# ltdoanh2004/MotionDiffusion-MoE

Hardware: AMD Instinct MI355X
Metric: denoising-steps/sec (B=32, T=196, 263-d, 8 experts) (higher is better)
Workload: dtype bf16; 1 GPU; configs[1]: model_size=small, num_experts=8, B=32/GPU, T=196, 1000-step DDPM with CFG 7.5 (cond+uncond batched as 64 rows), N_text=28, hipGraph=on, streams=1; global_batch=32, parallelism=batch-shard x1, weights replicated

## Files before the change

### include/mdm_hip.h

```cpp
#ifndef MDM_HIP_H
#define MDM_HIP_H
#include <stdint.h>

#ifdef __cplusplus
extern "C" {
#endif

enum { MDM_OK = 0, MDM_ERR_ARG = 1, MDM_ERR_LAUNCH = 2, MDM_ERR_UNSUPPORTED = 3 };
enum { MDM_OP_F32_ROW = 0, MDM_OP_F32_KSTRIDE = 1, MDM_OP_BF16_ROW = 2, MDM_OP_FP8_ROW = 3 ,
       MDM_OP_X2_ROW = 4 };
enum { MDM_ACT_NONE = 0, MDM_ACT_GELU = 1, MDM_ACT_SILU = 2, MDM_ACT_FEAT = 3,
       MDM_ACT_HEADNORM = 4,
       MDM_ACT_HEADSOFTMAX = 5 };
enum { MDM_H16_BF16 = 1, MDM_H16_F16 = 2 };
enum { MDM_PREC_BF16 = 1, MDM_PREC_F16 = 2, MDM_PREC_X3 = 3, MDM_PREC_MIXED = 4, MDM_PREC_FP8 = 5 };

typedef struct MdmOperand {
  const void* p;
  const void* p_lo;
  int64_t ld;
  int64_t gstride;
  const int32_t* gather;
  int64_t bs1, bs2;
  int32_t rpg;
// ... 378 lines not shown
  float* w1;
  float* b1;
  float* w2;
  float* b2;
  float* st_emb_w;
  float* st_emb_b;
  float* st_norm_w;
  float* st_norm_b;
  float* st_out_w;
  float* st_out_b;
} MdmMoeTensors;

int64_t mdm_moe_train_workspace_bytes(int32_t B, int32_t S, int32_t D, int32_t F, int32_t E, int32_t Te);
int mdm_moe_ffn_train_forward(const MdmMoeTensors* params, int32_t D, int32_t F, int32_t E, int32_t Te, int32_t De,
                              const float* eph_w, const float* eph_b, const float* x, const float* emb, int32_t B, int32_t S,
                              float dropout_p, uint64_t seed, float* out, float* lb_loss, int32_t* route_out, void* ws,
                              int64_t ws_bytes, void* stream);
int mdm_moe_ffn_train_backward(const MdmMoeTensors* params, int32_t D, int32_t F, int32_t E, int32_t Te, int32_t De,
                               const float* eph_w, const float* x, const float* emb, int32_t B, int32_t S, float dropout_p,
                               uint64_t seed, const float* dout, float* dx, float* demb, const MdmMoeTensors* grads, void* ws,
                               int64_t ws_bytes, void* stream);
int mdm_sumsq(const float* x, int64_t n, float* out, void* stream);
int mdm_adam_step(float* p, const float* g, float* m, float* v, int64_t n, float lr, float beta1, float beta2, float eps,
                  int32_t step, const float* sumsq, float max_norm, void* stream);

int mdm_xattn_gate(const float* gate, const float* adaptive_gate, int32_t D, float* out, void* stream);
int mdm_fill_i64(int64_t* dst, int64_t n, const int32_t* src_dev, void* stream);
int mdm_add_i32(int32_t* dst, int32_t delta, void* stream);

enum MdmVariant {
  MDM_VAR_DEFAULT = 0,
  MDM_VAR_GEMM_256 = 6,
  MDM_VAR_SD_UNFOLDED = 22,
  MDM_VAR_GENERIC_DH256 = 23,
  MDM_VAR_SD_FOLD_ANY = 24,
  MDM_VAR_ROUTER_CONST_E = 26,
  MDM_VAR_ROUTER_RUNTIME_E = 27,
  MDM_VAR_MLP_LDS = 34,
  MDM_VAR_TAIL_SPLIT = 35,
  MDM_VAR_X3_REG = 36,
  MDM_VAR_QKV_SPLIT = 50,
  MDM_VAR_XQ_SPLIT = 51,
  MDM_VAR_X3_ATTN_CHAIN = 52,
  MDM_VAR_X3_XATTN_CHAIN = 56,
  MDM_VAR_X3_STYLE_SPLIT = 60,
  MDM_VAR_X3_TAILS_SPLIT = 61,
  MDM_VAR_X3_F32_ROWS = 62,
  MDM_VAR_STREAM_NEVER = 63,
  MDM_VAR_STREAM_ALWAYS = 68,
  MDM_VAR_STREAM3_NEVER = 69,
  MDM_VAR_STREAM3_ALWAYS = 70
};
enum MdmRouteVariant { MDM_VAR_ROUTE_LAUNCH = 171 };
int mdm_set_gemm_variant(int variant);

int mdm_probe_enable(int32_t enable);
int mdm_route_dump(int32_t* buf, int64_t capacity);
int mdm_route_workspace(const MdmModel* m, int32_t B, int32_t T, int32_t N, int64_t* off);
int mdm_sd_fold_passes(int32_t D, int32_t H, int32_t N);
int mdm_probe_read(float* us, int32_t* rows, int32_t cap);


int64_t mdm_gru_bidir_workspace_bytes(int32_t B, int32_t H);
int mdm_gru_bidir(const float* gx, const float* w_hh, const float* b_hh, const float* h0, const int32_t* lens_dev,
                  const int32_t* lens_host, int32_t B, int32_t T, int32_t H, float* out, float* ws, int64_t ws_bytes, void* stream);
int mdm_eval_pad_rows(const float* src, int64_t ld_src, int32_t B, int32_t T, int32_t C, int32_t Cp, int32_t pad, int32_t leaky,
                      float* dst, void* stream);
int mdm_eval_ln_leaky(const float* x, int32_t M, int32_t N, const float* w, const float* b, float eps, float* y, void* stream);
int mdm_eval_matching(const float* text, const float* motion, int32_t B, int32_t D, float* dist, int32_t* rank, float* diag,
                      void* stream);
int mdm_eval_center(const float* x, int32_t N, int32_t D, float* mean, float* xc, void* stream);

const char* mdm_version(void);

#ifdef __cplusplus
}
#endif
#endif
```

### motiondiffusion-moe_amd/csrc/api.hip

```cpp
#include "gemm.h"
#include "kernels.h"

namespace mdm {
namespace {

__global__ void pack_bf16_kernel(const float* __restrict__ src, int64_t ld_src, int64_t rows, int64_t K,
                                 uint16_t* __restrict__ hi, uint16_t* __restrict__ lo, int64_t ld_dst) {
  const int64_t pairs_per_row = ld_dst >> 1;
  const int64_t total = rows * pairs_per_row;
  for (int64_t i = blockIdx.x * (int64_t)blockDim.x + threadIdx.x; i < total; i += (int64_t)gridDim.x * blockDim.x) {
    const int64_t r = i / pairs_per_row, k = (i - r * pairs_per_row) * 2;
    const float a = k < K ? src[r * ld_src + k] : 0.f;
    const float b = k + 1 < K ? src[r * ld_src + k + 1] : 0.f;
    uint32_t h, l;
    split_bf16(a, b, h, l);
    *(uint32_t*)(hi + r * ld_dst + k) = h;
    if (lo) *(uint32_t*)(lo + r * ld_dst + k) = l;
  }
}

__global__ void pack_f16_kernel(const float* __restrict__ src, int64_t ld_src, int64_t rows, int64_t K,
                                uint16_t* __restrict__ dst, int64_t ld_dst) {
  const int64_t pairs_per_row = ld_dst >> 1;
  const int64_t total = rows * pairs_per_row;
  for (int64_t i = blockIdx.x * (int64_t)blockDim.x + threadIdx.x; i < total; i += (int64_t)gridDim.x * blockDim.x) {
    const int64_t r = i / pairs_per_row, k = (i - r * pairs_per_row) * 2;
    const float a = k < K ? src[r * ld_src + k] : 0.f;
    const float b = k + 1 < K ? src[r * ld_src + k + 1] : 0.f;
    *(uint32_t*)(dst + r * ld_dst + k) = pack_f16(a, b);
  }
}

}
}

namespace mdm {
int g_variant = MDM_VAR_DEFAULT;
}

extern "C" {

int mdm_set_gemm_variant(int v) {
  switch (v) {
    case MDM_VAR_DEFAULT:
    case MDM_VAR_GEMM_256:
    case MDM_VAR_SD_UNFOLDED:
    case MDM_VAR_GENERIC_DH256:
    case MDM_VAR_SD_FOLD_ANY:
    case MDM_VAR_ROUTER_CONST_E:
    case MDM_VAR_ROUTER_RUNTIME_E:
    case MDM_VAR_MLP_LDS:
    case MDM_VAR_TAIL_SPLIT:
    case MDM_VAR_X3_REG:
    case MDM_VAR_QKV_SPLIT:
    case MDM_VAR_XQ_SPLIT:
    case MDM_VAR_X3_ATTN_CHAIN:
    case MDM_VAR_X3_XATTN_CHAIN:
    case MDM_VAR_X3_STYLE_SPLIT:
    case MDM_VAR_X3_TAILS_SPLIT:
    case MDM_VAR_X3_F32_ROWS:
    case MDM_VAR_STREAM_NEVER:
    case MDM_VAR_STREAM_ALWAYS:
    case MDM_VAR_STREAM3_NEVER:
    case MDM_VAR_STREAM3_ALWAYS:
    case MDM_VAR_ROUTE_LAUNCH:
      mdm::g_variant = v;
      return MDM_OK;
    default:
      return MDM_ERR_ARG;
  }
}

const char* mdm_version(void) { return "mdm_hip 0.1 (gfx950)"; }

int mdm_gemm(const MdmGemmDesc* d, void* stream) {
  if (!d) return MDM_ERR_ARG;
  return mdm::gemm(*d, (hipStream_t)stream);
}

int mdm_fused_mlp(const MdmMlpDesc* d, void* stream) {
  if (!d) return MDM_ERR_ARG;
  return mdm::fused_mlp(*d, (hipStream_t)stream);
}

int64_t mdm_mlp_stream_elems(int32_t G, int32_t F, int32_t Din, int32_t Dout) { return mdm::mlp_stream_elems(G, F, Din, Dout); }

int mdm_mlp_stream_pack(const float* w1, const float* w2, int32_t G, int32_t F, int32_t Din, int32_t Dout, int32_t h16,
                        uint16_t* out, void* stream) {
  return mdm::mlp_stream_pack(w1, w2, G, F, Din, Dout, h16, out, (hipStream_t)stream);
}

int64_t mdm_gemm_stream_elems(int32_t N, int32_t K) { return mdm::gemm_stream_elems(N, K); }

int mdm_gemm_stream_pack(const float* w, int32_t N, int32_t K, int32_t h16, uint16_t* out, void* stream) {
  return mdm::gemm_stream_pack(w, N, K, h16, out, (hipStream_t)stream);
}

int64_t mdm_gemm_stream1_elems(int32_t N, int32_t K) { return mdm::gemm_stream1_elems(N, K); }

int mdm_gemm_stream1_pack(const float* w, int64_t ldw, int32_t N, int32_t K, int32_t h16, uint16_t* out, void* stream) {
  return mdm::gemm_stream1_pack(w, ldw, N, K, h16, out, (hipStream_t)stream);
}

int64_t mdm_gemm_stream3x_elems(int32_t G, int32_t N, int32_t K) { return mdm::gemm_stream3x_elems(G, N, K); }

int64_t mdm_gemm_stream3x_group_elems(int32_t N, int32_t K) { return mdm::gemm_stream3x_group_elems(N, K); }

int mdm_gemm_stream3x_pack(const float* w, int64_t ldw, int32_t G, int32_t N, int32_t K, uint16_t* out, void* stream) {
  return mdm::gemm_stream3x_pack(w, ldw, G, N, K, out, (hipStream_t)stream);
}

int64_t mdm_gemm_stream3_elems(int32_t N, int32_t K) { return mdm::gemm_stream3_elems(N, K); }

int mdm_gemm_stream3_pack(const float* w, int32_t N, int32_t K, uint16_t* out, void* stream) {
  return mdm::gemm_stream3_pack(w, N, K, out, (hipStream_t)stream);
}

int mdm_pack_bf16(const float* src, int64_t ld_src, int64_t rows, int64_t K, uint16_t* hi, uint16_t* lo,
// ... 35 lines not shown
```

### motiondiffusion-moe_amd/csrc/gemm.h

```cpp
#pragma once
#include "mdm_common.h"
#include "mdm_hip.h"

namespace mdm {

typedef MdmOperand Operand;
typedef MdmGemmDesc GemmArgs;

enum OperandKind { OP_F32_ROW = MDM_OP_F32_ROW, OP_F32_KSTRIDE = MDM_OP_F32_KSTRIDE, OP_BF16_ROW = MDM_OP_BF16_ROW, OP_X2_ROW = MDM_OP_X2_ROW };
enum Act { ACT_NONE = MDM_ACT_NONE, ACT_GELU = MDM_ACT_GELU, ACT_SILU = MDM_ACT_SILU, ACT_FEAT = MDM_ACT_FEAT, ACT_HEADNORM = MDM_ACT_HEADNORM, ACT_HEADSOFTMAX = MDM_ACT_HEADSOFTMAX };

inline GemmArgs gemm_defaults(int precision) {
  GemmArgs g = {};
  g.batch = 1;
  g.nb2 = 1;
  g.alpha = 1.f;
  g.out_scale = 1.f;
  g.r1_scale = 1.f;
  g.precision = precision;
  g.a_scale_u = 1.f;
  g.c8_scale = 1.f;
  return g;
}
inline Operand op_f32(const float* p, int64_t ld) {
  Operand o = {};
  o.p = p;
  o.ld = ld;
  o.kind = OP_F32_ROW;
  return o;
}
inline Operand op_f32_kstride(const float* p, int64_t ld) {
  Operand o = {};
  o.p = p;
  o.ld = ld;
  o.kind = OP_F32_KSTRIDE;
  return o;
}
inline Operand op_bf16(const uint16_t* hi, const uint16_t* lo, int64_t ld) {
  Operand o = {};
  o.p = hi;
  o.p_lo = lo;
  o.ld = ld;
  o.kind = OP_BF16_ROW;
  return o;
}

int gemm(const GemmArgs& a, hipStream_t stream);
bool gemm_bf16_eligible(const GemmArgs& a);
int gemm_bf16(const GemmArgs& a, hipStream_t stream);
bool gemm_bf16_256_eligible(const GemmArgs& a);
int gemm_bf16_256(const GemmArgs& a, hipStream_t stream);
bool fused_mlp_supported(const MdmMlpDesc& a);
int fused_mlp(const MdmMlpDesc& a, hipStream_t stream);
bool gemm_x3_dma_eligible(const GemmArgs& a);
int gemm_x3_dma(const GemmArgs& a, hipStream_t stream);
bool gemm_fp8_eligible(const GemmArgs& a);
int gemm_fp8(const GemmArgs& a, hipStream_t stream);
int64_t gemm_stream1_elems(int N, int K);
int gemm_stream1_pack(const float* w, int64_t ldw, int N, int K, int h16, uint16_t* out, hipStream_t stream);
bool gemm_stream1_eligible(const GemmArgs& a);
bool gemm_stream1_wanted(const GemmArgs& a);
int gemm_stream1(const GemmArgs& a, hipStream_t stream);
int64_t gemm_stream3x_elems(int G, int N, int K);
int64_t gemm_stream3x_group_elems(int N, int K);
int gemm_stream3x_pack(const float* w, int64_t ldw, int G, int N, int K, uint16_t* out, hipStream_t stream);
bool gemm_stream3x_eligible(const GemmArgs& a);
bool gemm_stream3x_wanted(const GemmArgs& a);
int gemm_stream3x(const GemmArgs& a, hipStream_t stream);
bool fused_mlp_stream_supported(const MdmMlpDesc& a);
int fused_mlp_stream(const MdmMlpDesc& a, hipStream_t stream);
struct PairTail {
  const float *pw, *pb;
  const float *sw, *sb;
  const float* sc;
  int S;
  const uint16_t* ws;
  const float* bias;
  const float* resid;
  float out_scale;
  float* out;
  const float *lw, *lb;
  uint16_t* ln16;
  const float* skip;
  float skip_scale;
  const float *l2w, *l2b;
};
bool fused_pair_style_supported(const MdmMlpDesc& a);
int fused_pair_style(const MdmMlpDesc& a, const PairTail& t, hipStream_t stream);
int64_t mlp_stream_elems(int G, int F, int Din, int Dout);
int mlp_stream_pack(const float* w1, const float* w2, int G, int F, int Din, int Dout, int h16, uint16_t* out, hipStream_t stream);
int64_t gemm_stream_elems(int N, int K);
int gemm_stream_pack(const float* w, int N, int K, int h16, uint16_t* out, hipStream_t stream);
bool style_gemm_supported(int D, int64_t M);
int64_t gemm_stream3_elems(int N, int K);
int gemm_stream3_pack(const float* w, int N, int K, uint16_t* out, hipStream_t stream);
struct StyleTail3 {
  const float *lw = nullptr, *lb = nullptr;
  float* ln_out = nullptr;
  const float* skip = nullptr;
  float skip_scale = 0.f;
  const float *l2w = nullptr, *l2b = nullptr;
  int ln_x2 = 0;
};
struct MoeGateParams;
struct StyleRoute {
  const MoeGateParams* gate = nullptr;
  int E = 0;
  int* cursor = nullptr;
};
bool style_gemm_route_supported(int D, int64_t M, int E, int hn_fmt, int h16);
int64_t style_gemm_route_parts(int64_t M);
int style_gemm3(const float* src, int64_t M, int D, int S, const float* pw, const float* pb, const float* sw, const float* sb,
                const float* sc, const int* pos4, const uint16_t* ws3, const float* bias, const float* resid, float out_scale,
                const float* colscale, float* out, const StyleTail3& t, hipStream_t s);
int style_gemm(const void* src, int src_fmt, int64_t M, int D, int S, const float* pw, const float* pb, const float* sw, const float* sb,
               const float* sc, const int* pos4, const uint16_t* ws, const float* bias, const float* resid, float out_scale,
               const float* colscale, float* out, uint16_t* out16, int h16, hipStream_t s, const StyleRoute* route = nullptr);

}
```

### motiondiffusion-moe_amd/csrc/mlp_stream.hip

```cpp
#include <utility>

#include "gemm.h"
#include "kernels.h"
#include "row.h"

namespace mdm {
namespace {

constexpr int NT = 512, FC = 256;

template <typename T>
__device__ __forceinline__ T ldg(const uint8_t* p) {
  return *(const T*)p;
}

__device__ __forceinline__ void pin() { __builtin_amdgcn_sched_barrier(0); }

__device__ __forceinline__ void lds_barrier() {
  asm volatile("s_waitcnt lgkmcnt(0)" ::: "memory");
  __builtin_amdgcn_s_barrier();
  asm volatile("" ::: "memory");
}

__device__ __forceinline__ bool find_tile(const MdmMlpDesc& g, const int* gtab, int tile_h, int lane, int mt, int& row0, int& row_end,
// ... 243 lines not shown
    for (int i = 0; i < RT; ++i) {
      const int ml = i * 16 + frow;
      f32x4 v = y[i][j];
      v[0] = (v[0] + bb[0]) * st.out_scale, v[1] = (v[1] + bb[1]) * st.out_scale, v[2] = (v[2] + bb[2]) * st.out_scale,
      v[3] = (v[3] + bb[3]) * st.out_scale;
      *(f32x4*)(stg + ml * D + (((n >> 2) ^ (ml & 31)) << 2)) = v;
    }
  }
  lds_barrier();
  {
    R8 xr[RPW], sk[RPW];
#pragma unroll
    for (int q = 0; q < RPW; ++q) {
      int64_t m = (int64_t)row0 + RPW * wn + q;
      m = m < row_end ? m : row_end - 1;
      xr[q].load(st.resid + m * D, D, lane);
      if (st.skip) sk[q].load(st.skip + m * D, D, lane);
    }
    R8 lww, lbb, l2ww, l2bb;
    if (st.lw) lww.load(st.lw, D, lane), lbb.load(st.lb, D, lane);
    if (st.l2w) l2ww.load(st.l2w, D, lane), l2bb.load(st.l2b, D, lane);
#pragma unroll
    for (int q = 0; q < RPW; ++q) {
      const int rl = RPW * wn + q;
      const int64_t m = (int64_t)row0 + rl;
      if (m >= row_end) continue;
      R8 r;
      const R8& x = xr[q];
      const f32x4 v0 = *(const f32x4*)(stg + rl * D + ((lane ^ (rl & 31)) << 2));
      const f32x4 v1 = *(const f32x4*)(stg + rl * D + (((64 + lane) ^ (rl & 31)) << 2));
      r.e[0] = v0[0] + x.e[0], r.e[1] = v0[1] + x.e[1], r.e[2] = v0[2] + x.e[2], r.e[3] = v0[3] + x.e[3];
      r.e[4] = v1[0] + x.e[4], r.e[5] = v1[1] + x.e[5], r.e[6] = v1[2] + x.e[6], r.e[7] = v1[3] + x.e[7];
      if (st.skip) {
#pragma unroll
        for (int j = 0; j < 8; ++j) r.e[j] = sk[q].e[j] + st.skip_scale * r.e[j];
        r.layernorm(lww, lbb, D, lane);
        r.store(st.out + m * D, D, lane);
        if (st.l2w) {
          r.layernorm(l2ww, l2bb, D, lane);
          r.template store_h16<FMT>(st.ln16 + m * D, D, lane);
        }
      } else {
        r.store(st.out + m * D, D, lane);
        if (st.ln16) {
          r.layernorm(lww, lbb, D, lane);
          r.template store_h16<FMT>(st.ln16 + m * D, D, lane);
        }
      }
    }
  }
}

template <typename HT, int RT, int NJ, int DIN, int TAIL>
__global__ __launch_bounds__(NT, 2) void fused_mlp_stream_kernel(const MdmMlpDesc g, const int tile_h, const PairTail st) {
  typedef typename HT::frag_t frag_t;
  static_assert(!TAIL || (NJ == 4 && DIN == 512 && RT <= 4), "the tail is written for D = 512 rows");
  typedef XGeo<RT, DIN, NJ, TAIL != 0> G;
  constexpr int NKO = DIN / 128, NLINE = DIN / 64;
  constexpr int NA = 4, PD = NA - 1;
  constexpr int NR = (RT <= 4 && NJ == 4 && DIN % 256 == 0) ? 16 : 8;
  constexpr int NF = 4 * RT;
  static_assert(NF % NA == 0, "the ring must close over the unrolled body");
  extern __shared__ __attribute__((aligned(1024))) uint8_t smem[];
  uint8_t* const ximg = smem;
  uint8_t* const hid = smem + G::XIMG_B;
  int* const gtab = (int*)(smem + G::SMEM);
  {
    const int ng = g.goff ? g.ngroups : 1;
    if ((int)threadIdx.x <= ng) gtab[threadIdx.x] = g.goff ? g.goff[threadIdx.x] : (threadIdx.x ? g.M : 0);
    lds_barrier();
  }

  for (int mt = xcd_remap(blockIdx.x, gridDim.x);; mt += gridDim.x) {
    int tid = threadIdx.x;
    asm volatile("" : "+v"(tid));
    const int lane = tid & 63;
    const int wn = __builtin_amdgcn_readfirstlane(tid >> 6);
    int row0, row_end, grp;
    if (!find_tile(g, gtab, tile_h, lane, mt, row0, row_end, grp)) break;

    const int nchunk = g.F / FC;
    constexpr int fpc = (DIN / 32) * 2 + 8 * NJ;
    const uint8_t* wp = (const uint8_t*)g.wstream + ((int64_t)grp * g.wstream_gs + (int64_t)wn * nchunk * fpc * 512) * 2 + lane * 16;

    frag_t R[NR];
#pragma unroll
    for (int f = 0; f < NR; ++f) R[f] = ldg<frag_t>(wp + f * 1024);
    wp += NR * 1024;

    if (wn < RT) {
      const uint8_t* xp[2];
#pragma unroll
      for (int hf = 0; hf < 2; ++hf) {
        const int r = 16 * wn + 8 * hf + (lane >> 3);
        int srow = row0 + r;
        srow = srow < row_end ? srow : row_end - 1;
        const int64_t src = g.gather ? (int64_t)g.gather[srow] : (int64_t)srow;
        xp[hf] = (const uint8_t*)(g.X + src * g.ldx) + (lane & 7) * 16;
      }
      constexpr int LB = NLINE < 8 ? NLINE : 8;
#pragma unroll
      for (int c0 = 0; c0 < NLINE; c0 += LB) {
        uint4 v[2][LB];
#pragma unroll
        for (int c = 0; c < LB; ++c)
#pragma unroll
          for (int hf = 0; hf < 2; ++hf) v[hf][c] = ldg<uint4>(xp[hf] + (c0 + c) * 128);
#pragma unroll
        for (int c = 0; c < LB; ++c)
#pragma unroll
          for (int hf = 0; hf < 2; ++hf) {
            const int r = 16 * wn + 8 * hf + (lane >> 3);
            const int ch = (8 * (c0 + c) + (lane & 7)) ^ (r & 15);
            *(uint4*)(ximg + r * G::XROW_B + (ch << 4)) = v[hf][c];
          }
      }
    }
    f32x4 y[RT][NJ];
    {
      const float* b2 = g.b2 ? g.b2 + (int64_t)grp * g.b2_gs + wn * (16 * NJ) + (lane >> 4) * 4 : nullptr;
#pragma unroll
      for (int j = 0; j < NJ; ++j) {
        const f32x4 bb = b2 ? *(const f32x4*)(b2 + j * 16) : (f32x4){0.f, 0.f, 0.f, 0.f};
#pragma unroll
        for (int i = 0; i < RT; ++i) y[i][j] = bb;
      }
// ... 74 lines not shown
              R[s0 + 1] = ldg<frag_t>(wp + (s0 + 1) * 1024);
            }
            pin();
          }
        }
        wp += NR * 1024;
      }
    };
    auto publish = [&](int ln) __attribute__((always_inline)) {
      const int fr = ln & 15;
      uint8_t* const hw = hid + fr * 256 + (((2 * wn + (ln >> 5)) ^ fr) << 4) + ((ln >> 4) & 1) * 8;
      lds_barrier();
#pragma unroll
      for (int i = 0; i < RT; ++i) *(uint2*)(hw + i * 4096) = pk[i];
      lds_barrier();
    };
    auto olane = [&]() __attribute__((always_inline)) {
      int ln = lane;
      asm volatile("" : "+v"(ln));
      return ln;
    };
    auto hbase = [](int ln) { return (ln & 15) * 256 + ((((ln >> 4) ^ (ln & 15))) << 4); };

    {
      const int ln = olane();
      phase1(0, ln);
      gelu_alone(I0());
      publish(ln);
      phase2(I0(), hbase(ln));
      gelu_alone(I1());
      publish(ln);
    }
#pragma unroll 1
    for (int chunk = 1; chunk < nchunk; ++chunk) {
      const int ln = olane();
      phase1(chunk, ln);
      phase2(I1(), hbase(ln));
      gelu_alone(I0());
      publish(ln);
      phase2(I0(), hbase(ln));
      gelu_alone(I1());
      publish(ln);
    }
    phase2(I1(), hbase(olane()));

    int te = threadIdx.x;
    asm volatile("" : "+v"(te));
    if constexpr (TAIL) {
      pair_tail<HT, RT, NR>(st, y, R, smem, row0, row_end, te, wn);
    } else {
      store_tile<HT, RT, NJ, G::SMEM>(g, y, smem, row0, row_end, te, wn, te & 15, (te & 63) >> 4);
    }
    lds_barrier();
  }
}

template <typename HT>
__global__ __launch_bounds__(256) void mlp_stream_pack_kernel(const float* w1, const float* w2, int G, int F, int Din, int Dout,
                                                              uint16_t* out) {
  const int NJ = Dout / 128, nchunk = F / FC, f1 = 2 * (Din / 32), q = 4 * NJ, fpc = f1 + 2 * q;
  const int64_t nfrag = (int64_t)G * 8 * nchunk * fpc;
  for (int64_t fi = (int64_t)blockIdx.x * 4 + (threadIdx.x >> 6); fi < nfrag; fi += (int64_t)gridDim.x * 4) {
    const int l = threadIdx.x & 63;
    const int f = (int)(fi % ((int64_t)nchunk * fpc));
    const int w = (int)((fi / ((int64_t)nchunk * fpc)) % 8);
    const int gi = (int)(fi / ((int64_t)nchunk * fpc) / 8);
    int c, loc;
    if (f < f1 + q) {
      c = 0, loc = f;
    } else {
      c = 1 + (f - (f1 + q)) / fpc, loc = (f - (f1 + q)) % fpc;
    }
    const float* src;
    int hh = -1, cc = c, fp = 0;
    if (c == nchunk) {
      hh = 1, cc = nchunk - 1, fp = loc;
    } else if (loc >= f1) {
      if (c == 0) hh = 0, fp = loc - f1;
      else if (loc < f1 + q) hh = 1, cc = c - 1, fp = loc - f1;
      else hh = 0, fp = loc - f1 - q;
    }
    if (hh < 0) {
      const int step = loc >> 1, j = loc & 1;
      src = w1 + ((int64_t)gi * F + 256 * c + 32 * w + 16 * j + (l & 15)) * Din + 32 * step + 8 * (l >> 4);
    } else {
      const int s = fp / NJ, j = fp % NJ, p = 32 * s + 8 * (l >> 4);
      src = w2 + ((int64_t)gi * Dout + 16 * NJ * w + 16 * j + (l & 15)) * F + 256 * cc + 32 * (p >> 4) + 16 * hh + (p & 15);
    }
    uint4 o;
    o.x = HT::pack(src[0], src[1]), o.y = HT::pack(src[2], src[3]), o.z = HT::pack(src[4], src[5]), o.w = HT::pack(src[6], src[7]);
    *(uint4*)(out + fi * 512 + l * 8) = o;
  }
}

int device_cus() {
  static int cus[64] = {};
  const int dev = dev_ordinal();
  if (!cus[dev]) {
    int n = 0;
    if (hipDeviceGetAttribute(&n, hipDeviceAttributeMultiprocessorCount, dev) != hipSuccess || n <= 0) n = 256;
    cus[dev] = n;
  }
  return cus[dev];
}

}
// ... 33 lines not shown
  int64_t h = (M + cus * rounds - 1) / (cus * rounds);
  h = (h + 15) & ~15ll;
  if (h < 16) h = 16;
  if (h > rt_max * 16) h = rt_max * 16;
  return (int)h;
}

template <int RT, int DIN, int TAIL, int NJ = 4>
static int launch_stream(const MdmMlpDesc& a, int th, hipStream_t stream, const PairTail& tail = PairTail()) {
  constexpr int smem = XGeo<RT, DIN, NJ, TAIL != 0>::SMEM + 512;
  static DevOnce attr;
  if (smem > 65536 && !attr) {
    if (hipFuncSetAttribute((const void*)fused_mlp_stream_kernel<HB, RT, NJ, DIN, TAIL>, hipFuncAttributeMaxDynamicSharedMemorySize, smem) != hipSuccess ||
        hipFuncSetAttribute((const void*)fused_mlp_stream_kernel<HF, RT, NJ, DIN, TAIL>, hipFuncAttributeMaxDynamicSharedMemorySize, smem) != hipSuccess)
      return MDM_ERR_LAUNCH;
    attr = true;
  }
  const int tiles = (int)(a.M / th) + (a.goff ? a.ngroups : 1);
  const int res = device_cus();
  const int grid = tiles < res ? tiles : res;
  if (a.h16 == MDM_H16_F16) {
    hipLaunchKernelGGL((fused_mlp_stream_kernel<HF, RT, NJ, DIN, TAIL>), dim3(grid), dim3(NT), smem, stream, a, th, tail);
  } else {
    hipLaunchKernelGGL((fused_mlp_stream_kernel<HB, RT, NJ, DIN, TAIL>), dim3(grid), dim3(NT), smem, stream, a, th, tail);
  }
  MDM_RETURN_IF_LAUNCH_FAILED();
  return MDM_OK;
}

template <int DIN>
static int launch_by_height(const MdmMlpDesc& a, hipStream_t stream) {
  const int th = mlp_stream_tile_h(a.M, 7);
  if (th <= 32) return launch_stream<2, DIN, 0>(a, th, stream);
  if (th <= 64) return launch_stream<4, DIN, 0>(a, th, stream);
  return launch_stream<7, DIN, 0>(a, th, stream);
}

int fused_mlp_stream(const MdmMlpDesc& a, hipStream_t stream) {
  if (!a.X || (!a.C && !a.C16)) return MDM_ERR_ARG;
  if (!fused_mlp_stream_supported(a)) return MDM_ERR_UNSUPPORTED;
  if (a.Dout == 1024) {
    const int th = mlp_stream_tile_h(a.M, 4);
    return launch_stream<4, 1024, 0, 8>(a, th, stream);
  }
  if (a.Din == 128) return launch_by_height<128>(a, stream);
  if (a.Din == 256) return launch_by_height<256>(a, stream);
  return launch_by_height<512>(a, stream);
}

bool fused_pair_style_supported(const MdmMlpDesc& a) {
  return fused_mlp_stream_supported(a) && a.Din == 512 && a.Dout == 512 && !a.goff && !a.gather && !a.rowscale && !a.R1 && !a.R2;
}

int fused_pair_style(const MdmMlpDesc& a, const PairTail& t, hipStream_t stream) {
  if (!a.X || !fused_pair_style_supported(a)) return MDM_ERR_UNSUPPORTED;
  if (!t.pw || !t.pb || !t.sw || !t.sb || !t.sc || t.S <= 0 || !t.ws || !t.bias || !t.resid || !t.out || (t.ln16 && (!t.lw || !t.lb)) ||
      ((uintptr_t)t.ws & 15) || (t.skip && (!t.lw || !t.lb)) || (t.l2w && (!t.l2b || !t.ln16 || !t.skip)))
    return MDM_ERR_ARG;
  const int th = mlp_stream_tile_h(a.M, 4);
  if (th <= 32) return launch_stream<2, 512, 1>(a, th, stream, t);
  return launch_stream<4, 512, 1>(a, th, stream, t);
}

}
```

### motiondiffusion-moe_amd/csrc/model.hip

```cpp
#include "gemm.h"
#include "kernels.h"

namespace mdm {
namespace {

#define MDM_TRY(expr)            \
  do {                           \
    int st__ = (expr);           \
    if (st__ != MDM_OK) return st__; \
  } while (0)

constexpr int PROBE_MAX = 64;
struct Probe {
  bool on = false;
  int n = 0;
  hipEvent_t a[PROBE_MAX], b[PROBE_MAX];
  int rows[PROBE_MAX];
  bool made = false;
};
Probe g_probe;
bool probe_armed() { return g_probe.on && g_probe.n < PROBE_MAX; }
int probe_begin(hipStream_t s) { return probe_armed() && hipEventRecord(g_probe.a[g_probe.n], s) != hipSuccess ? MDM_ERR_LAUNCH : MDM_OK; }
int probe_end(hipStream_t s, int rows) {
  if (!probe_armed()) return MDM_OK;
// ... 199 lines not shown
  const int D = c.m->D;
  const StylePath path = style_path(c, st, src_bf16, out16 != nullptr, t3 != nullptr);
  if (route && path != StylePath::FUSED16) return MDM_ERR_UNSUPPORTED;
  switch (path) {
    case StylePath::FUSED16:
      return style_gemm(src, src_bf16 ? c.h16 : 0, c.M, D, c.S, pw, pb, st.norm_w, st.norm_b, sc, pos4, st.out_ws, st.out_b, resid,
                        out_scale, colscale, out, out16, c.h16, c.s, route);
    case StylePath::FUSED3:
    case StylePath::FUSED3_TAIL:
      return style_gemm3(src, c.M, D, c.S, pw, pb, st.norm_w, st.norm_b, sc, pos4, st.out_ws3, st.out_b, resid, out_scale, colscale, out,
                         path == StylePath::FUSED3_TAIL ? *t3 : StyleTail3(), c.s);
    case StylePath::SPLIT: {
      MDM_TRY(style_in(src, c.M, D, c.S, pw, pb, st.norm_w, st.norm_b, sc, pos4, src_bf16 ? c.h16 : 0, tmp, fmt16(c), c.s));
      LinOpts o;
      o.out_scale = out_scale, o.R1 = resid, o.colscale = colscale;
      return linear(c, act_of(c, tmp), c.M, D, st.out, st.out_b, D, out, out16, o);
    }
  }
}

MdmMlpDesc proj_pair_desc(const Ctx& c, const MdmPerformer& p) {
  const int D = c.m->D;
  MdmMlpDesc f = {};
  f.X = (const uint16_t*)c.w.t4, f.ldx = D, f.M = (int)c.M, f.Din = D, f.F = D, f.Dout = D;
  f.b1 = p.proj0_b, f.b2 = p.proj3_b, f.wstream = p.proj_ws, f.wstream_gs = 2 * (int64_t)D * D;
  f.r1_scale = 1.f, f.C16 = (uint16_t*)c.w.t4, f.ldc = D, f.h16 = c.h16;
  return f;
}
enum class ProjPath { PAIR_TAIL, PAIR, LINEARS_X2, LINEARS };
ProjPath proj_path(const Ctx& c, const MdmPerformer& p) {
  if (c.bf && p.proj_ws) {
    const MdmMlpDesc f = proj_pair_desc(c, p);
    if (p.style.out_ws && g_variant != MDM_VAR_TAIL_SPLIT && fused_pair_style_supported(f)) return ProjPath::PAIR_TAIL;
    if (fused_mlp_stream_supported(f)) return ProjPath::PAIR;
  }
  return x2_rows(c) ? ProjPath::LINEARS_X2 : ProjPath::LINEARS;
}

enum class PerfCore { CORE3, CORE256, CORE16_QKV, CORE16, CHAIN };
PerfCore perf_core_path(const Ctx& c, const MdmPerformer& p, bool xn16) {
  const int D = c.m->D, H = c.m->H, dh = D / H;
  if (c.bf && g_variant != MDM_VAR_GENERIC_DH256 && perf_attn256_supported(dh, c.S) &&
      perf_attn256_scratch_bytes(c.B, H, c.S) <= c.M * 2 * D * (int64_t)sizeof(float))
    return PerfCore::CORE256;
  if (c.bf && perf_attn_supported(dh, c.S))
    return xn16 && g_variant != MDM_VAR_QKV_SPLIT && perf_attn_qkv_supported(dh, c.S, H) ? PerfCore::CORE16_QKV : PerfCore::CORE16;
  if (x3_flow(c) && !xn16 && g_variant != MDM_VAR_X3_ATTN_CHAIN && perf_attn3_supported(dh, c.S) && D % 32 == 0 && p.qkv.lo &&
      p.feat.lo && (c.M * 3 * D) % 8 == 0)
    return PerfCore::CORE3;
  return PerfCore::CHAIN;
}

int performer(const Ctx& c, const MdmPerformer& p, const float* x, Act xn, const float* sc, float* out,
              const StyleTail3& pt = StyleTail3()) {
  const MdmModel& m = *c.m;
  const int D = m.D, H = m.H, dh = D / H, mf = dh;
  const Work& w = c.w;
  LinOpts qo;
  qo.alpha = 0.1f;
  Act att = act_of(c, w.t4);
  switch (perf_core_path(c, p, xn.bf)) {
    case PerfCore::CORE3: {
      uint16_t* const xh = (uint16_t*)w.qkv;
      uint16_t* const xl = xh + c.M * 3 * D;
      GemmArgs g = planes_gemm(c, xn, p.qkv, p.qkv_b, 3 * D, xh, xl);
      g.alpha = 0.1f, g.act = ACT_HEADNORM, g.hn_w = p.hn_w, g.hn_b = p.hn_b, g.hn_l2_tiles = 2 * H;
      MDM_TRY(gemm(g, c.s));
      MDM_TRY(perf_attn3(xh, xl, p.feat.hi, p.feat.lo, (int)p.feat.ld, p.hn_w, p.hn_b, c.len, c.B, c.S, H, dh, w.t4, c.x2 ? 1 : 0, c.s));
      att.x2 = c.x2;
      break;
    }
    case PerfCore::CORE256:
      MDM_TRY(linear(c, xn, c.M, D, p.qkv, p.qkv_b, 3 * D, nullptr, (uint16_t*)w.qkv, qo));
      MDM_TRY(perf_attn256(w.qkv, c.h16, p.feat.hi, (int)p.feat.ld, p.hn_w, p.hn_b, c.len, c.B, c.S, H, (uint16_t*)w.t4, w.phi, c.s));
      break;
    case PerfCore::CORE16_QKV:
      MDM_TRY(perf_attn_qkv((const uint16_t*)xn.p, p.qkv.hi, (int)p.qkv.ld, p.qkv_b, 0.1f, (uint16_t*)w.qkv, c.h16, p.feat.hi,
                            (int)p.feat.ld, p.hn_w, p.hn_b, c.len, c.B, c.S, H, dh, (uint16_t*)w.t4, c.s));
      break;
    case PerfCore::CORE16:
      MDM_TRY(linear(c, xn, c.M, D, p.qkv, p.qkv_b, 3 * D, nullptr, (uint16_t*)w.qkv, qo));
      MDM_TRY(perf_attn(w.qkv, c.h16, p.feat.hi, (int)p.feat.ld, p.hn_w, p.hn_b, c.len, c.B, c.S, H, dh, (uint16_t*)w.t4, c.s));
      break;
    case PerfCore::CHAIN: {
      MDM_TRY(linear(c, xn, c.M, D, p.qkv, p.qkv_b, 3 * D, w.qkv, nullptr, qo));
      MDM_TRY(head_norm(w.qkv, c.M, H, dh, p.hn_w, p.hn_b, c.s));
      const bool f16p = c.bf && c.h16 == MDM_H16_F16 && !p.feat.lo;
      Operand P = packed(p.feat);
      if (f16p) {
        const int64_t pn = (int64_t)mf * p.feat.ld;
        if (pn > (int64_t)c.B * H * dh * dh) return MDM_ERR_UNSUPPORTED;
        uint16_t* const ph = (uint16_t*)w.kvt;
        MDM_TRY(f16_to_bf16x2(p.feat.hi, pn, ph, ph + pn, c.s));
        P = op_bf16(ph, ph + pn, p.feat.ld);
      }
      const int cprec = f16p ? 3 : c.prec;
      GemmArgs g = gd(c);
      g.precision = cprec;
      g.A = op_f32(w.qkv, dh);
      g.A.rpg = 2 * H, g.A.gstride = 3 * D;
      g.W = P;
      g.M = (int)(c.M * 2 * H), g.N = mf, g.K = dh;
      g.C = w.phi, g.ldc = mf;
      g.act = ACT_FEAT;
      g.feat_len = c.len, g.feat_S = c.S, g.feat_rpt = 2 * H, g.feat_kslot = H;
      MDM_TRY(gemm(g, c.s));
      GemmArgs kv = per_head(c, heads(op_f32_kstride(w.qkv + 2 * D, 3 * D), (int64_t)c.S * 3 * D, dh),
                             heads(op_f32_kstride(w.phi + H * mf, 2 * H * mf), (int64_t)c.S * 2 * H * mf, mf), dh, mf, c.S, mf,
                             (int64_t)H * dh * mf, (int64_t)dh * mf);
      kv.C = w.kvt, kv.out_scale = 0.1f, kv.precision = cprec;
      MDM_TRY(gemm(kv, c.s));
      GemmArgs num = per_head(c, heads(op_f32(w.phi, 2 * H * mf), (int64_t)c.S * 2 * H * mf, mf),
                              heads(op_f32(w.kvt, mf), (int64_t)H * dh * mf, (int64_t)dh * mf), c.S, dh, mf, D, (int64_t)c.S * D, dh);
      num.C = w.t2, num.out_scale = 0.1f, num.precision = cprec;
      MDM_TRY(gemm(num, c.s));
      MDM_TRY(den_ln(w.t2, w.phi, c.M, H, dh, p.hn_w, p.hn_b, w.t4, fmt16(c), c.s));
      break;
    }
  }
  switch (proj_path(c, p)) {
    case ProjPath::PAIR_TAIL: {
      PairTail t = {};
      t.pw = p.post_w, t.pb = p.post_b, t.sw = p.style.norm_w, t.sb = p.style.norm_b, t.sc = sc, t.S = c.S;
      t.ws = p.style.out_ws, t.bias = p.style.out_b, t.resid = x, t.out_scale = 0.1f, t.out = out;
      t.lw = pt.lw, t.lb = pt.lb, t.ln16 = (uint16_t*)pt.ln_out, t.skip = pt.skip, t.skip_scale = pt.skip_scale, t.l2w = pt.l2w, t.l2b = pt.l2b;
      return fused_pair_style(proj_pair_desc(c, p), t, c.s);
    }
    case ProjPath::PAIR:
      MDM_TRY(fused_mlp_stream(proj_pair_desc(c, p), c.s));
      break;
    case ProjPath::LINEARS_X2: {
      LinOpts o;
      o.act = ACT_GELU, o.outx2 = (uint16_t*)w.t2;
      MDM_TRY(linear(c, att, c.M, D, p.proj0, p.proj0_b, D, nullptr, nullptr, o));
      MDM_TRY(linear(c, Act{w.t2, false, true}, c.M, D, p.proj3, p.proj3_b, D, w.t4, nullptr));
      break;
    }
    case ProjPath::LINEARS: {
      LinOpts o;
      o.act = ACT_GELU;
      MDM_TRY(linear_to_act(c, att, c.M, D, p.proj0, p.proj0_b, D, w.t2, o));
      MDM_TRY(linear_to_act(c, act_of(c, w.t2), c.M, D, p.proj3, p.proj3_b, D, w.t4));
      break;
    }
  }
  const bool tail3 = !c.bf && (pt.ln_out || pt.skip);
  return style_apply(c, p.style, w.t4, p.post_w, p.post_b, nullptr, sc, w.t2, x, 0.1f, nullptr, out, nullptr, c.bf,
                     tail3 ? &pt : nullptr);
}

enum class DualTail { NONE, T16, T3 };
DualTail dual_tail_path(const Ctx& c, const MdmLayer& l) {
  if (proj_path(c, l.local) == ProjPath::PAIR_TAIL && proj_path(c, l.global) == ProjPath::PAIR_TAIL) return DualTail::T16;
  if (style_path(c, l.local.style, false, false, true) == StylePath::FUSED3_TAIL &&
      style_path(c, l.global.style, false, false, true) == StylePath::FUSED3_TAIL)
    return DualTail::T3;
  return DualTail::NONE;
}

int dual_block(const Ctx& c, const MdmLayer& l, const float* x, const uint16_t* x16, const float* sc4, float* out,
               const float* next_w = nullptr, const float* next_b = nullptr) {
  const int D = c.m->D;
  const Work& w = c.w;
  const int64_t scs = (int64_t)c.B * 2 * D;
  const int xnf = fmt_xn(c);
  const Act xa = c.bf ? act_bf16(x16) : act_f32(x);
  LinOpts so;
  so.act = ACT_GELU;
  switch (dual_tail_path(c, l)) {
    case DualTail::T16:
    case DualTail::T3: {
      MDM_TRY(linear(c, xa, c.M, D, l.skip, l.skip_b, D, w.f1, nullptr, so));
      MDM_TRY(ln_chain(x, c.M, D, l.dual_pre_w, l.dual_pre_b, w.t1, 0, l.local.pre_w, l.local.pre_b, w.t3, xnf, c.s));
      StyleTail3 pt;
      pt.lw = l.global.pre_w, pt.lb = l.global.pre_b, pt.ln_out = w.t3, pt.ln_x2 = c.x2;
      MDM_TRY(performer(c, l.local, w.t1, act_x2(c, w.t3), sc4 + 0 * scs, w.t5, pt));
      StyleTail3 bt;
      bt.skip = w.f1, bt.skip_scale = 0.1f, bt.lw = l.dual_post_w, bt.lb = l.dual_post_b;
      if (next_w) bt.l2w = next_w, bt.l2b = next_b, bt.ln_out = w.t2, bt.ln_x2 = c.x2;
      return performer(c, l.global, w.t5, act_x2(c, w.t3), sc4 + 1 * scs, out, bt);
    }
    case DualTail::NONE: {
      MDM_TRY(ln_chain(x, c.M, D, l.dual_pre_w, l.dual_pre_b, w.t1, 0, l.local.pre_w, l.local.pre_b, w.t3, xnf, c.s));
      const bool normed = proj_path(c, l.local) == ProjPath::PAIR_TAIL;
      StyleTail3 pt;
      if (normed) pt.lw = l.global.pre_w, pt.lb = l.global.pre_b, pt.ln_out = w.t3;
      MDM_TRY(performer(c, l.local, w.t1, act_x2(c, w.t3), sc4 + 0 * scs, w.t5, pt));
      if (!normed) MDM_TRY(ln_chain(w.t5, c.M, D, l.global.pre_w, l.global.pre_b, w.t3, xnf, nullptr, nullptr, nullptr, 0, c.s));
      MDM_TRY(performer(c, l.global, w.t5, act_x2(c, w.t3), sc4 + 1 * scs, w.t1));
      so.R1 = w.t1, so.r1_scale = 0.1f;
      MDM_TRY(linear(c, xa, c.M, D, l.skip, l.skip_b, D, w.t3, nullptr, so));
      return ln_chain(w.t3, c.M, D, l.dual_post_w, l.dual_post_b, out, 0, next_w, next_b, next_w ? w.t2 : nullptr, xnf, c.s);
    }
  }
}

enum class XattnPath { CORE3, CORE_Q, CORE, CHAIN };
XattnPath lin_xattn_path(const Ctx& c, const MdmLayer& l) {
  const int D = c.m->D, H = c.m->H, dh = D / H;
  if (c.bf && lin_xattn_supported(dh) && !(dh == 256 && g_variant == MDM_VAR_GENERIC_DH256))
    return g_variant != MDM_VAR_XQ_SPLIT && D == 512 && lin_xattn_q_supported(dh, c.S, H) ? XattnPath::CORE_Q : XattnPath::CORE;
  if (x3_flow(c) && g_variant != MDM_VAR_X3_XATTN_CHAIN && xattn3_supported(dh, 1) && l.ca_q.lo && D % 32 == 0 && (c.M * D) % 8 == 0)
    return XattnPath::CORE3;
  return XattnPath::CHAIN;
}

enum class RoutePath { FOLDED, LAUNCH };
RoutePath route_path(const Ctx& c, const MdmLayer& l) {
  if (g_variant == MDM_VAR_ROUTE_LAUNCH || g_variant == MDM_VAR_ROUTER_CONST_E || g_variant == MDM_VAR_ROUTER_RUNTIME_E) return RoutePath::LAUNCH;
  if (c.bf && !c.fp8 && style_path(c, l.ca_style, true, false, false) == StylePath::FUSED16 &&
      style_gemm_route_supported(c.m->D, c.M, c.m->E, fmt_mlp(c), c.h16))
    return RoutePath::FOLDED;
  return RoutePath::LAUNCH;
}
MoeGateParams gate_params(const Ctx& c, const MdmLayer& l, const int* forced) {
  const Work& w = c.w;
  MoeGateParams p = {};
  for (int b = 0; b < 2; ++b) {
    p.ln_w[b] = l.moe_ln_w[b], p.ln_b[b] = l.moe_ln_b[b];
    p.gate_w[b] = l.gate_w[b], p.gate_b[b] = l.gate_b[b];
    p.usage[b] = l.usage[b], p.importance[b] = l.importance[b];
  }
  p.hn = w.hn, p.hn_bf16 = c.fp8 ? 3 : fmt_mlp(c), p.hn_scale = w.hn_scale, p.top_idx = w.top_idx, p.top_val = w.top_val, p.hist = w.hist, p.uimp = w.uimp, p.forced_idx = forced;
  return p;
}

int cross_block(const Ctx& c, const MdmLayer& l, const float* at, const float* x, const float* sc, float* out,
                bool pre_normed = false, const StyleRoute* route = nullptr) {
  const MdmModel& m = *c.m;
// ... 720 lines not shown
```

Baseline: 240.8 denoising-steps/sec.

## Ride the dual-block skip GEMM on idle CUs of the pair-tail kernel

Adds a combined kernel where the first workgroups run the fused pair-style MLP tiles and extra workgroups on otherwise idle CUs compute the skip linear with GELU into the skip buffer. The dual block offers this rider to the local performer and falls back to a separate skip GEMM launch when the rider cannot run. This removes one kernel launch and fills CUs left idle by the tile kernel. In exchange the kernel uses max(tile, rider) shared memory, which may lower occupancy, and the skip GEMM becomes a less tuned hand-written path.

New measurement: 246.1 denoising-steps/sec (median of 6 runs). +2.2%, better.

```diff
diff --git a/include/mdm_hip.h b/include/mdm_hip.h
--- a/include/mdm_hip.h
+++ b/include/mdm_hip.h
@@ -454,6 +454,7 @@
   MDM_VAR_STREAM3_ALWAYS = 70
 };
 enum MdmRouteVariant { MDM_VAR_ROUTE_LAUNCH = 171 };
+enum MdmSkipVariant { MDM_VAR_SKIP_LAUNCH = 172 };
 int mdm_set_gemm_variant(int variant);
 
 int mdm_probe_enable(int32_t enable);
diff --git a/motiondiffusion-moe_amd/csrc/api.hip b/motiondiffusion-moe_amd/csrc/api.hip
--- a/motiondiffusion-moe_amd/csrc/api.hip
+++ b/motiondiffusion-moe_amd/csrc/api.hip
@@ -64,6 +64,7 @@
     case MDM_VAR_STREAM3_NEVER:
     case MDM_VAR_STREAM3_ALWAYS:
     case MDM_VAR_ROUTE_LAUNCH:
+    case MDM_VAR_SKIP_LAUNCH:
       mdm::g_variant = v;
       return MDM_OK;
     default:
diff --git a/motiondiffusion-moe_amd/csrc/gemm.h b/motiondiffusion-moe_amd/csrc/gemm.h
--- a/motiondiffusion-moe_amd/csrc/gemm.h
+++ b/motiondiffusion-moe_amd/csrc/gemm.h
@@ -69,6 +69,16 @@
 int gemm_stream3x(const GemmArgs& a, hipStream_t stream);
 bool fused_mlp_stream_supported(const MdmMlpDesc& a);
 int fused_mlp_stream(const MdmMlpDesc& a, hipStream_t stream);
+struct SkipRider {
+  const uint16_t* X;
+  int64_t ldx;
+  const uint16_t* W;
+  int64_t ldw;
+  const float* bias;
+  float* C;
+  int64_t ldc;
+  int M;
+};
 struct PairTail {
   const float *pw, *pb;
   const float *sw, *sb;
@@ -84,9 +94,10 @@
   const float* skip;
   float skip_scale;
   const float *l2w, *l2b;
+  const SkipRider* rider;
 };
 bool fused_pair_style_supported(const MdmMlpDesc& a);
-int fused_pair_style(const MdmMlpDesc& a, const PairTail& t, hipStream_t stream);
+int fused_pair_style(const MdmMlpDesc& a, const PairTail& t, hipStream_t stream, bool* rode = nullptr);
 int64_t mlp_stream_elems(int G, int F, int Din, int Dout);
 int mlp_stream_pack(const float* w1, const float* w2, int G, int F, int Din, int Dout, int h16, uint16_t* out, hipStream_t stream);
 int64_t gemm_stream_elems(int N, int K);
diff --git a/motiondiffusion-moe_amd/csrc/mlp_stream.hip b/motiondiffusion-moe_amd/csrc/mlp_stream.hip
--- a/motiondiffusion-moe_amd/csrc/mlp_stream.hip
+++ b/motiondiffusion-moe_amd/csrc/mlp_stream.hip
@@ -319,7 +319,7 @@
 }
 
 template <typename HT, int RT, int NJ, int DIN, int TAIL>
-__global__ __launch_bounds__(NT, 2) void fused_mlp_stream_kernel(const MdmMlpDesc g, const int tile_h, const PairTail st) {
+__device__ __forceinline__ void mlp_stream_tiles(const MdmMlpDesc& g, const int tile_h, const PairTail& st, const int wg, const int nwg) {
   typedef typename HT::frag_t frag_t;
   static_assert(!TAIL || (NJ == 4 && DIN == 512 && RT <= 4), "the tail is written for D = 512 rows");
   typedef XGeo<RT, DIN, NJ, TAIL != 0> G;
@@ -338,7 +338,7 @@
     lds_barrier();
   }
 
-  for (int mt = xcd_remap(blockIdx.x, gridDim.x);; mt += gridDim.x) {
+  for (int mt = xcd_remap(wg, nwg);; mt += nwg) {
     int tid = threadIdx.x;
     asm volatile("" : "+v"(tid));
     const int lane = tid & 63;
@@ -519,6 +519,111 @@
       store_tile<HT, RT, NJ, G::SMEM>(g, y, smem, row0, row_end, te, wn, te & 15, (te & 63) >> 4);
     }
     lds_barrier();
+  }
+}
+
+template <typename HT, int RT, int NJ, int DIN, int TAIL>
+__global__ __launch_bounds__(NT, 2) void fused_mlp_stream_kernel(const MdmMlpDesc g, const int tile_h, const PairTail st) {
+  mlp_stream_tiles<HT, RT, NJ, DIN, TAIL>(g, tile_h, st, blockIdx.x, gridDim.x);
+}
+
+constexpr int RIDER_RT = 7, RIDER_ROWS = RIDER_RT * 16, RIDER_SMEM = RIDER_ROWS * 1024;
+
+template <typename HT>
+__device__ __forceinline__ void skip_rider(const SkipRider& rd, const int r, const int nr) {
+  typedef typename HT::frag_t frag_t;
+  extern __shared__ __attribute__((aligned(1024))) uint8_t smem[];
+  constexpr int RT = RIDER_RT, NR = 16, AHEAD = NR / 4;
+  const int items = (rd.M + RIDER_ROWS - 1) / RIDER_ROWS;
+#pragma unroll 1
+  for (int it = r; it < items; it += nr) {
+    int tid = threadIdx.x;
+    asm volatile("" : "+v"(tid));
+    const int lane = tid & 63, frow = lane & 15, fq = lane >> 4;
+    const int wn = __builtin_amdgcn_readfirstlane(tid >> 6);
+    const int row0 = it * RIDER_ROWS;
+    const uint8_t* const wp = (const uint8_t*)(rd.W + (int64_t)(wn * 64 + frow) * rd.ldw + 8 * fq);
+    const int64_t jst = 32 * rd.ldw;
+    frag_t R[NR];
+#pragma unroll
+    for (int f = 0; f < NR; ++f) R[f] = ldg<frag_t>(wp + (f & 3) * jst + (f >> 2) * 64);
+
+    if (wn < RT) {
+      const uint8_t* xp[2];
+#pragma unroll
+      for (int hf = 0; hf < 2; ++hf) {
+        int srow = row0 + 16 * wn + 8 * hf + (lane >> 3);
+        srow = srow < rd.M ? srow : rd.M - 1;
+        xp[hf] = (const uint8_t*)(rd.X + (int64_t)srow * rd.ldx) + (lane & 7) * 16;
+      }
+      uint4 v[2][8];
+#pragma unroll
+      for (int c = 0; c < 8; ++c)
+#pragma unroll
+        for (int hf = 0; hf < 2; ++hf) v[hf][c] = ldg<uint4>(xp[hf] + c * 128);
+#pragma unroll
+      for (int c = 0; c < 8; ++c)
+#pragma unroll
+        for (int hf = 0; hf < 2; ++hf) {
+          const int rr = 16 * wn + 8 * hf + (lane >> 3);
+          const int ch = (8 * c + (lane & 7)) ^ (rr & 15);
+          *(uint4*)(smem + rr * 1024 + (ch << 4)) = v[hf][c];
+        }
+    }
+    f32x4 y[RT][4];
+#pragma unroll
+    for (int i = 0; i < RT; ++i)
+#pragma unroll
+      for (int j = 0; j < 4; ++j) y[i][j] = (f32x4){0.f, 0.f, 0.f, 0.f};
+    lds_barrier();
+    {
+      const int xb = frow * 1024 + ((fq ^ frow) << 4);
+      frag_t A[2][RT];
+#pragma unroll
+      for (int i = 0; i < RT; ++i) A[0][i] = *(const frag_t*)(smem + xb + i * 16384);
+#pragma unroll
+      for (int s = 0; s < 16; ++s) {
+        if (s + 1 < 16) {
+#pragma unroll
+          for (int i = 0; i < RT; ++i) A[(s + 1) & 1][i] = *(const frag_t*)(smem + (xb ^ (64 * ((s + 1) & 3))) + ((s + 1) >> 2) * 256 + i * 16384);
+        }
+        const int sn = s + AHEAD < 16 ? s + AHEAD : 15;
+#pragma unroll
+        for (int j = 0; j < 4; ++j) {
+          const int slot = (s * 4 + j) & (NR - 1);
+#pragma unroll
+          for (int i = 0; i < RT; ++i) y[i][j] = HT::mfma16(R[slot], A[s & 1][i], y[i][j]);
+          R[slot] = ldg<frag_t>(wp + j * jst + sn * 64);
+        }
+        pin();
+      }
+    }
+    int te = threadIdx.x;
+    asm volatile("" : "+v"(te));
+    const int er = te & 15, eq = (te & 63) >> 4;
+#pragma unroll
+    for (int j = 0; j < 4; ++j) {
+      const int n = wn * 64 + 16 * j + 4 * eq;
+      const f32x4 bb = *(const f32x4*)(rd.bias + n);
+#pragma unroll
+      for (int i = 0; i < RT; ++i) {
+        const int m = row0 + i * 16 + er;
+        const f32x2 a = gelu_erf2((f32x2){y[i][j][0] + bb[0], y[i][j][1] + bb[1]});
+        const f32x2 b = gelu_erf2((f32x2){y[i][j][2] + bb[2], y[i][j][3] + bb[3]});
+        if (m < rd.M) *(f32x4*)(rd.C + (int64_t)m * rd.ldc + n) = (f32x4){a[0] + 0.f, a[1] + 0.f, b[0] + 0.f, b[1] + 0.f};
+      }
+    }
+    lds_barrier();
+  }
+}
+
+template <typename HT, int RT>
+__global__ __launch_bounds__(NT, 2) void pair_tail_rider_kernel(const MdmMlpDesc g, const int tile_h, const PairTail st, const SkipRider rd,
+                                                                const int ntile_wg) {
+  if ((int)blockIdx.x < ntile_wg) {
+    mlp_stream_tiles<HT, RT, 4, 512, 1>(g, tile_h, st, blockIdx.x, ntile_wg);
+  } else {
+    skip_rider<HT>(rd, (int)blockIdx.x - ntile_wg, (int)gridDim.x - ntile_wg);
   }
 }
 
@@ -658,12 +763,56 @@
   return fused_mlp_stream_supported(a) && a.Din == 512 && a.Dout == 512 && !a.goff && !a.gather && !a.rowscale && !a.R1 && !a.R2;
 }
 
-int fused_pair_style(const MdmMlpDesc& a, const PairTail& t, hipStream_t stream) {
+template <int RT>
+static int launch_riders(const MdmMlpDesc& a, int th, hipStream_t stream, const PairTail& tail, int ntile_wg, int riders) {
+  constexpr int tile_smem = XGeo<RT, 512, 4, true>::SMEM + 512;
+  constexpr int smem = tile_smem > RIDER_SMEM ? tile_smem : RIDER_SMEM;
+  static_assert(smem <= 160 * 1024, "one CU's LDS");
+  static DevOnce attr;
+  if (!attr) {
+    if (hipFuncSetAttribute((const void*)pair_tail_rider_kernel<HB, RT>, hipFuncAttributeMaxDynamicSharedMemorySize, smem) != hipSuccess ||
+        hipFuncSetAttribute((const void*)pair_tail_rider_kernel<HF, RT>, hipFuncAttributeMaxDynamicSharedMemorySize, smem) != hipSuccess)
+      return MDM_ERR_LAUNCH;
+    attr = true;
+  }
+  if (a.h16 == MDM_H16_F16) {
+    hipLaunchKernelGGL((pair_tail_rider_kernel<HF, RT>), dim3(ntile_wg + riders), dim3(NT), smem, stream, a, th, tail, *tail.rider, ntile_wg);
+  } else {
+    hipLaunchKernelGGL((pair_tail_rider_kernel<HB, RT>), dim3(ntile_wg + riders), dim3(NT), smem, stream, a, th, tail, *tail.rider, ntile_wg);
+  }
+  MDM_RETURN_IF_LAUNCH_FAILED();
+  return MDM_OK;
+}
+
+static int rider_count(const MdmMlpDesc& a, int th, const SkipRider& r, int& ntile_wg) {
+  const int cus = device_cus();
+  const int tiles = a.M / th + 1;
+  ntile_wg = tiles < cus ? tiles : cus;
+  if (!r.X || !r.W || !r.bias || !r.C || r.M < 1 || (r.ldx % 8) || (r.ldw % 8) || r.ldw < 512 || (r.ldc & 3) ||
+      ((((uintptr_t)r.X) | ((uintptr_t)r.W) | ((uintptr_t)r.bias) | ((uintptr_t)r.C)) & 15))
+    return 0;
+  const int items = (r.M + RIDER_ROWS - 1) / RIDER_ROWS;
+  const int riders = cus - ntile_wg < items ? cus - ntile_wg : items;
+  if (riders < 1 || (items + riders - 1) / riders > 2) return 0;
+  return riders;
+}
+
+int fused_pair_style(const MdmMlpDesc& a, const PairTail& t, hipStream_t stream, bool* rode) {
+  if (rode) *rode = false;
   if (!a.X || !fused_pair_style_supported(a)) return MDM_ERR_UNSUPPORTED;
   if (!t.pw || !t.pb || !t.sw || !t.sb || !t.sc || t.S <= 0 || !t.ws || !t.bias || !t.resid || !t.out || (t.ln16 && (!t.lw || !t.lb)) ||
       ((uintptr_t)t.ws & 15) || (t.skip && (!t.lw || !t.lb)) || (t.l2w && (!t.l2b || !t.ln16 || !t.skip)))
     return MDM_ERR_ARG;
   const int th = mlp_stream_tile_h(a.M, 4);
+  if (t.rider && rode) {
+    int ntile_wg;
+    const int riders = rider_count(a, th, *t.rider, ntile_wg);
+    if (riders) {
+      const int rc = th <= 32 ? launch_riders<2>(a, th, stream, t, ntile_wg, riders) : launch_riders<4>(a, th, stream, t, ntile_wg, riders);
+      *rode = rc == MDM_OK;
+      return rc;
+    }
+  }
   if (th <= 32) return launch_stream<2, 512, 1>(a, th, stream, t);
   return launch_stream<4, 512, 1>(a, th, stream, t);
 }
diff --git a/motiondiffusion-moe_amd/csrc/model.hip b/motiondiffusion-moe_amd/csrc/model.hip
--- a/motiondiffusion-moe_amd/csrc/model.hip
+++ b/motiondiffusion-moe_amd/csrc/model.hip
@@ -275,7 +275,8 @@
 }
 
 int performer(const Ctx& c, const MdmPerformer& p, const float* x, Act xn, const float* sc, float* out,
-              const StyleTail3& pt = StyleTail3()) {
+              const StyleTail3& pt = StyleTail3(), const SkipRider* rider = nullptr, bool* rode = nullptr) {
+  if (rode) *rode = false;
   const MdmModel& m = *c.m;
   const int D = m.D, H = m.H, dh = D / H, mf = dh;
   const Work& w = c.w;
@@ -347,7 +348,8 @@
       t.pw = p.post_w, t.pb = p.post_b, t.sw = p.style.norm_w, t.sb = p.style.norm_b, t.sc = sc, t.S = c.S;
       t.ws = p.style.out_ws, t.bias = p.style.out_b, t.resid = x, t.out_scale = 0.1f, t.out = out;
       t.lw = pt.lw, t.lb = pt.lb, t.ln16 = (uint16_t*)pt.ln_out, t.skip = pt.skip, t.skip_scale = pt.skip_scale, t.l2w = pt.l2w, t.l2b = pt.l2b;
-      return fused_pair_style(proj_pair_desc(c, p), t, c.s);
+      t.rider = rider;
+      return fused_pair_style(proj_pair_desc(c, p), t, c.s, rode);
     }
     case ProjPath::PAIR:
       MDM_TRY(fused_mlp_stream(proj_pair_desc(c, p), c.s));
@@ -390,14 +392,19 @@
   const Act xa = c.bf ? act_bf16(x16) : act_f32(x);
   LinOpts so;
   so.act = ACT_GELU;
-  switch (dual_tail_path(c, l)) {
+  const DualTail path = dual_tail_path(c, l);
+  switch (path) {
     case DualTail::T16:
     case DualTail::T3: {
-      MDM_TRY(linear(c, xa, c.M, D, l.skip, l.skip_b, D, w.f1, nullptr, so));
+      const bool offer = path == DualTail::T16 && g_variant != MDM_VAR_SKIP_LAUNCH;
+      const SkipRider sr = {x16, D, l.skip.hi, l.skip.ld, l.skip_b, w.f1, D, (int)c.M};
+      bool rode = false;
+      if (!offer) MDM_TRY(linear(c, xa, c.M, D, l.skip, l.skip_b, D, w.f1, nullptr, so));
       MDM_TRY(ln_chain(x, c.M, D, l.dual_pre_w, l.dual_pre_b, w.t1, 0, l.local.pre_w, l.local.pre_b, w.t3, xnf, c.s));
       StyleTail3 pt;
       pt.lw = l.global.pre_w, pt.lb = l.global.pre_b, pt.ln_out = w.t3, pt.ln_x2 = c.x2;
-      MDM_TRY(performer(c, l.local, w.t1, act_x2(c, w.t3), sc4 + 0 * scs, w.t5, pt));
+      MDM_TRY(performer(c, l.local, w.t1, act_x2(c, w.t3), sc4 + 0 * scs, w.t5, pt, offer ? &sr : nullptr, &rode));
+      if (offer && !rode) MDM_TRY(linear(c, xa, c.M, D, l.skip, l.skip_b, D, w.f1, nullptr, so));
       StyleTail3 bt;
       bt.skip = w.f1, bt.skip_scale = 0.1f, bt.lw = l.dual_post_w, bt.lb = l.dual_post_b;
       if (next_w) bt.l2w = next_w, bt.l2b = next_b, bt.ln_out = w.t2, bt.ln_x2 = c.x2;
```
